# darrenjw/logreg

Hardware: AMD Instinct MI355X
Metric: MCMC iterations/sec x chains for HMC (L=50) on n=200,p=8 (higher is better)
Workload: dtype f32

## Files before the change

logreg_amd/csrc/lr_engine.h:

```cpp
#pragma once

namespace {

template <typename T, int P> lr::ModelArgs<T, P> model_args(const lr_model* m) {
    lr::ModelArgs<T, P> a{};
    a.rows = static_cast<const T*>(m->d_rows);
    a.rows_tw = static_cast<const float*>(m->d_rows_tw);
    a.rows_mf = static_cast<const float*>(m->d_xmf);
    a.ops_mf = static_cast<const unsigned char*>(m->d_xms);
    a.n = m->n;
    for (int j = 0; j < P; ++j) a.prior.inv_var[j] = (T)m->inv_var[j];
    a.prior.lprior_const = m->lprior_const;
    return a;
}

int64_t plan_count(const lr_run_opts* o) { return o->plan_chains > 0 ? (int64_t)o->plan_chains : o->n_chains; }

struct RunSpec {
    int kind;
    double step;
    int l;
    double a[kMaxP], b[kMaxP], c[kMaxP];
};

// ... 48 lines not shown
    const int64_t head = pl.split > 0 ? (pl.split - pos0 < 0 ? 0 : (pl.split - pos0 > C ? C : pl.split - pos0)) : C;
    const bool two = head > 0 && head < C;
    const int64_t head_rounds = pl.mode == lr::MODE_MFMA ? head / ((pl.G == 1 ? 64 : 16) * (int64_t)m->cus) : head * pl.G / 64 / (4LL * m->cus);
    const bool both = two && pl.corun && (rs.kind != lr::KIND_HMC || head_rounds <= 2);
    lr_model::Side* side_slot = nullptr;
    if (both) {
        for (auto& e : m->sides)
            if (e.caller == st) side_slot = &e;
        if (!side_slot) {
            lr_model::Side e{st, nullptr, nullptr, nullptr};
            const bool ok = hipStreamCreateWithFlags(&e.stream, hipStreamNonBlocking) == hipSuccess &&
                            hipEventCreateWithFlags(&e.ev_fork, hipEventDisableTiming) == hipSuccess &&
                            hipEventCreateWithFlags(&e.ev_join, hipEventDisableTiming) == hipSuccess;
            if (!ok) {
                const hipError_t err = hipGetLastError();
                if (e.ev_join) (void)hipEventDestroy(e.ev_join);
                if (e.ev_fork) (void)hipEventDestroy(e.ev_fork);
                if (e.stream) (void)hipStreamDestroy(e.stream);
                return fail(LR_ERR_HIP, "creating the side stream of a two-part launch failed: %s", hipGetErrorString(err));
            }
            m->sides.push_back(e);
            side_slot = &m->sides.back();
        }
        if (hipEventRecord(side_slot->ev_fork, st) != hipSuccess || hipStreamWaitEvent(side_slot->stream, side_slot->ev_fork, 0) != hipSuccess)
            return fail(LR_ERR_HIP, "forking the two-part launch failed: %s", hipGetErrorString(hipGetLastError()));
    }
    for (int part = 0; part < 2; ++part) {
        ca.first = part == 0 ? 0 : head;
        ca.count = part == 0 ? head : C - head;
        if (ca.count <= 0) continue;
        const bool side = both && part == 1;
        lr::LaunchCfg cfg{part == 0 ? pl.mode : pl.mode2, part == 0 ? pl.G : pl.G2, part == 0 ? pl.R : pl.R2, rs.kind, side ? side_slot->stream : st,
                          part == 0 || pl.mode2 == lr::MODE_MIXED ? pl.lds_bytes : 0, m->dbg.residency_cap && !side ? m->cus : 0};
        const int rc = m->table->launch_chain(&cfg, ca.count, &ma, &ca);
        if (rc != 0) return fail(rc == -3 ? LR_ERR_UNSUPPORTED : LR_ERR_HIP, "chain launch failed (%d): %s", rc,
                                 hipGetErrorString(hipGetLastError()));
    }
    if (both) {
        if (hipEventRecord(side_slot->ev_join, side_slot->stream) != hipSuccess || hipStreamWaitEvent(st, side_slot->ev_join, 0) != hipSuccess)
            return fail(LR_ERR_HIP, "joining the two-part launch failed: %s", hipGetErrorString(hipGetLastError()));
    }
    return LR_OK;
}

template <typename T, int P>
int setup_tall(lr_model* m, const Plan& pl, hipStream_t st, int64_t C, int64_t Cp, lr::TallArgs<T, P>* pa) {
    lr::TallArgs<T, P>& a = *pa;
    a = lr::TallArgs<T, P>{};
    const int RS = pl.G;
    auto align = [](size_t b) { return (b + 255) & ~(size_t)255; };
    const size_t vec = align((size_t)C * P * sizeof(T)), dbl = align((size_t)C * sizeof(double));
    const InteriorPlan ip = plan_interior(m, Cp);
    const int RS_i = ip.RS_i, rs_waves = ip.waves;
    const int64_t slice_len_i = ip.slice_len_i;
    const int RSmax = RS_i > RS ? RS_i : RS;
    const size_t pg = align((size_t)RSmax * C * P * sizeof(T)), cv = align((size_t)2 * P * sizeof(T));
    const size_t need = 4 * vec + 2 * dbl + align((size_t)C * 4) + pg + align((size_t)RS * C * sizeof(double)) +
                        (RS_i > 0 && (m->P > 32 || rs_waves == 16) ? 2 * vec + pg : 0) + cv;
    lr_model::Ws* slot = nullptr;
    for (auto& e : m->ws)
        if (e.stream == st) slot = &e;
    if (!slot) {
        if (m->ws.size() >= 16) {
            if (hipDeviceSynchronize() != hipSuccess) return fail(LR_ERR_HIP, "hipDeviceSynchronize failed");
            for (auto& e : m->ws)
                if (e.p) (void)hipFree(e.p);
            m->ws.clear();
// ... 254 lines not shown
```

logreg_amd/csrc/lr_kernels.h:

```cpp
#pragma once
#include <type_traits>

#include "lr_device.h"
#include "lr_stamps.h"

namespace lr {

enum Kind { KIND_RWMH = 0, KIND_MALA = 1, KIND_HMC = 2, KIND_UL = 3 };
enum Mode { MODE_REG = 0, MODE_LDS = 1, MODE_GLOBAL = 2, MODE_MFMA = 3, MODE_STEPWISE = 4, MODE_MIXED = 5 };

template <typename T, int P> struct ModelArgs {
    const T* rows;
    const float* rows_tw;
    const float* rows_mf;
    const unsigned char* ops_mf;
    int64_t n;
    Prior<T, P> prior;
};

template <typename T> struct EvalArgs {
    const T* beta;
    int64_t C;
    int p;
    T* ll;
    T* lprior;
    T* lpost;
    T* grad;
};

template <typename T, int P> struct ChainArgs {
    T* state;
    double* lp_state;
    T* out;
    uint32_t* accepts;
    int64_t C;
    int64_t first, count;
    int64_t chain_offset;
    int64_t iters, thin;
    int64_t iter_offset;
    uint64_t seed;
    int p;
    int l;
    T step;
    T a[P], b[P], c[P];
    T d[P], e[P];
    StatsArgs stats;
    int interior_bf16;
};

template <typename T, int P, int G, int MODE, int R> struct RowsOf {
    using type = StridedRows<T, P, G>;
};
template <typename T, int P, int G, int R> struct RowsOf<T, P, G, MODE_REG, R> {
    using type = RegRows<T, P, R, G>;
};
template <int P, int G, int R> struct RowsOf<float, P, G, MODE_REG, R> {
    using type = RegRowPairs<P, R, G>;
};
template <typename T, int P, int R> struct RowsOf<T, P, 1, MODE_GLOBAL, R> {
    using type = ScalarRows<T, P>;
};
template <int R> struct RowsOf<float, 4, 1, MODE_GLOBAL, R> { using type = ScalarRowPairs<4>; };
template <int R> struct RowsOf<float, 8, 1, MODE_GLOBAL, R> { using type = ScalarRowPairs<8>; };
template <int R> struct RowsOf<float, 16, 1, MODE_GLOBAL, R> { using type = ScalarRowPairs<16>; };

template <typename T, int P, int G, int MODE, int R>
__device__ __forceinline__ typename RowsOf<T, P, G, MODE, R>::type make_rows(const ModelArgs<T, P>& m, int gl,
                                                                             T* smem) {
    typename RowsOf<T, P, G, MODE, R>::type rows;
    if constexpr (MODE == MODE_REG) {
        rows.load(m.rows, m.n, gl);
    } else if constexpr (MODE == MODE_LDS) {
        constexpr int LD = P + kLdsRowPad<T>;
        const int64_t tot = m.n * P;
        for (int64_t i = threadIdx.x; i < tot; i += blockDim.x) smem[(i / P) * LD + (i % P)] = m.rows[i];
        __syncthreads();
        rows.base = smem;
        rows.n = m.n;
        rows.gl = gl;
        rows.ld = LD;
// ... 775 lines not shown
```

logreg_amd/csrc/lr_mfma.h:

```cpp
#pragma once
#include <type_traits>

#include "lr_kernels.h"

namespace lr {

typedef float f32x4 __attribute__((ext_vector_type(4)));

typedef float mf_f32x2 __attribute__((ext_vector_type(2)));
typedef __bf16 mf_bf16x2 __attribute__((ext_vector_type(2)));
typedef __bf16 mf_bf16x8 __attribute__((ext_vector_type(8)));
typedef short mf_s16x4 __attribute__((ext_vector_type(4)));
typedef uint32_t mf_u32x2 __attribute__((ext_vector_type(2)));
typedef uint32_t mf_u32x4 __attribute__((ext_vector_type(4)));
__device__ __forceinline__ uint32_t mf_pack_rne(float a, float b) {
    return __builtin_bit_cast(uint32_t, __builtin_convertvector(mf_f32x2{a, b}, mf_bf16x2));
}
__device__ __forceinline__ float mf_hi_f32(uint32_t packed) { return __builtin_bit_cast(float, packed << 16); }

template <int P, typename Src> __device__ __forceinline__ float mf_row_or_zero(const Src* __restrict__ rows, int64_t n, int64_t row, int coord) {
    const float v = (float)rows[(row < n ? row : n - 1) * P + coord];
    return row < n ? v : 0.0f;
}

template <int P> constexpr int mf_image_floats();
template <int P, int S, bool VALUE>
__device__ __forceinline__ void mf_eval_stream(const float* __restrict__ rows, const float* __restrict__ image, int64_t n, int wave, int lane,
                                               int ntile_live, const float (&q)[P / 4], float (&gl)[P / 4], float& vsum) {
    constexpr int NC = P / 4, NG = (NC + 3) / 4, HG = NC < 4 ? NC : 4;
    const int c = lane & 15, k = lane >> 4;
    const int rp = c & 3, kp = c >> 2;
    float bs[NC];
#pragma unroll
    for (int h = 0; h < NC; ++h) bs[h] = q[h] * ExpScale<float>::k;
    f32x4 ga[NG], gb[NG];
#pragma unroll
    for (int g = 0; g < NG; ++g) ga[g] = gb[g] = f32x4{0, 0, 0, 0};
    float v = 0.0f;
    int pad = 0;
    constexpr int TB = P <= 8 ? 4 : 2;
// ... 49 lines not shown
                    ga[g] = __builtin_amdgcn_mfma_f32_16x16x4f32(cg[i][g][2], w[2], ga[g], 0, 0, 0);
                    gb[g] = __builtin_amdgcn_mfma_f32_16x16x4f32(cg[i][g][3], w[3], gb[g], 0, 0, 0);
                }
            }
        }
#pragma unroll
        for (int i = 0; i < TB; ++i) {
#pragma unroll
            for (int h = 0; h < NC; ++h) ca[i][h] = na[i][h];
#pragma unroll
            for (int g = 0; g < NG; ++g)
#pragma unroll
                for (int s2 = 0; s2 < 4; ++s2) cg[i][g][s2] = ng[i][g][s2];
        }
    }
#pragma unroll
    for (int h = 0; h < NC; ++h) gl[h] = ga[h >> 2][h & 3] + gb[h >> 2][h & 3];
    if constexpr (VALUE) vsum = (v + (float)pad) * ExpScale<float>::inv;
}

template <int P, int NTW, int S, bool END_MEM = false> struct MfmaRows {
    static constexpr int NC = P / 4;
    static constexpr int NU = NC / 2;
    static constexpr int NG = (NC + 3) / 4;
    static constexpr int HG = NC < 4 ? NC : 4;
    float xa[END_MEM ? 1 : NTW][NC];
    float xg[END_MEM ? 1 : NTW][NG][4];
    const float* rows_ = nullptr;
    const float* image = nullptr;
    int64_t n_ = 0;
    int wave_ = 0, lane_ = 0;
    int pad_rows;
    static constexpr int NPAIR = (NTW + 1) / 2;
    mf_u32x4 xe[NTW][NU];
    mf_u32x4 xq[NPAIR][NU];
    int ntile_live;

    template <typename Src> __device__ __forceinline__ void load(const Src* __restrict__ rows, int64_t n, int wave, int lane) {
        const int c = lane & 15, k = lane >> 4;
        const int rp = c & 3, kp = c >> 2;
        pad_rows = 0;
        if constexpr (END_MEM) {
            if constexpr (std::is_same<Src, float>::value) rows_ = rows;
            n_ = n;
            wave_ = wave;
            lane_ = lane;
        } else {
#pragma unroll
            for (int t = 0; t < NTW; ++t) {
                const int64_t base = 16 * ((int64_t)t * S + wave);
                const int64_t ra = base + c;
#pragma unroll
                for (int h = 0; h < NC; ++h) xa[t][h] = mf_row_or_zero<P>(rows, n, ra, k + 4 * h);
#pragma unroll
                for (int s = 0; s < 4; ++s) {
                    const int64_t rg = base + 4 * k + s;
#pragma unroll
                    for (int g = 0; g < NG; ++g) xg[t][g][s] = rp < HG ? mf_row_or_zero<P>(rows, n, rg, kp + 4 * (rp < HG ? rp : 0) + 16 * g) : 0.0f;
                    if (rg >= n) ++pad_rows;
                }
            }
        }
        auto piece = [&](int64_t row, int coord, int lo) {
            const float x = mf_row_or_zero<P>(rows, n, row, coord);
            const uint32_t h = mf_pack_rne(x, x) & 0xFFFFu;
            if (!lo) return h;
            return mf_pack_rne(x - mf_hi_f32(h), 0.0f) & 0xFFFFu;
        };
        ntile_live = 0;
#pragma unroll
        for (int t = 0; t < NTW; ++t) {
            const int64_t base = 16 * ((int64_t)t * S + wave);
            if (base < n) ntile_live = t + 1;
#pragma unroll
            for (int u = 0; u < NU; ++u) {
                uint32_t hl[2];
#pragma unroll
                for (int h = 0; h < 2; ++h) {
                    const float xs = mf_row_or_zero<P>(rows, n, base + c, k + 8 * u + 4 * h) * ExpScale<float>::k;
                    const uint32_t hi = mf_pack_rne(xs, xs) & 0xFFFFu;
                    hl[h] = hi | (mf_pack_rne(0.0f, xs - mf_hi_f32(hi)) & 0xFFFF0000u);
                }
                xe[t][u] = mf_u32x4{hl[0], hl[0], hl[1], hl[1]};
            }
        }
        const int grp = c >> 2, el = c & 3;
        const int gcoord = grp + 4 * (el >> 1), glo = el & 1;
#pragma unroll
        for (int pi = 0; pi < NPAIR; ++pi) {
#pragma unroll
            for (int u = 0; u < NU; ++u) {
                uint32_t v[8];
#pragma unroll
                for (int sl = 0; sl < 8; ++sl) {
                    const int t = 2 * pi + (sl >> 2);
                    const int64_t row = 16 * ((int64_t)t * S + wave) + 4 * k + (sl & 3);
                    v[sl] = t < NTW ? piece(row, gcoord + 8 * u, glo) : 0u;
                }
                xq[pi][u] = mf_u32x4{v[0] | (v[1] << 16), v[2] | (v[3] << 16), v[4] | (v[5] << 16), v[6] | (v[7] << 16)};
            }
        }
    }

    template <int NPL> __device__ __forceinline__ void eval_bf16(const float (&q)[NC], float (&gl)[NC]) const {
        static_assert(NPL >= 1 && NPL <= NPAIR, "pairs");
        mf_u32x4 bb[NU];
#pragma unroll
        for (int u = 0; u < NU; ++u) {
            const uint32_t ha = mf_pack_rne(q[2 * u], q[2 * u]), hb = mf_pack_rne(q[2 * u + 1], q[2 * u + 1]);
            const float la = q[2 * u] - mf_hi_f32(ha), lb = q[2 * u + 1] - mf_hi_f32(hb);
            bb[u] = mf_u32x4{ha, mf_pack_rne(la, la), hb, mf_pack_rne(lb, lb)};
        }
        constexpr int NT = 2 * NPL < NTW ? 2 * NPL : NTW;
        auto eta = [&](int t) {
            f32x4 acc = {0, 0, 0, 0};
#pragma unroll
            for (int u = 0; u < NU; ++u)
                acc = __builtin_amdgcn_mfma_f32_16x16x32_bf16(__builtin_bit_cast(mf_bf16x8, xe[t][u]), __builtin_bit_cast(mf_bf16x8, bb[u]), acc, 0, 0, 0);
            return acc;
        };
        f32x4 e[2 * NPL];
        e[0] = eta(0);
        if constexpr (NT > 1) e[1] = eta(1);
        if constexpr (S == 1) __builtin_amdgcn_sched_barrier(0);
        f32x4 gacc[NU];
#pragma unroll
        for (int u = 0; u < NU; ++u) gacc[u] = f32x4{0, 0, 0, 0};
#pragma unroll
        for (int pi = 0; pi < NPL; ++pi) {
            uint32_t wq[4] = {0u, 0u, 0u, 0u};
            if (2 * pi + 2 < NT) e[2 * pi + 2] = eta(2 * pi + 2);
            if (2 * pi + 3 < NT) e[2 * pi + 3] = eta(2 * pi + 3);
            if constexpr (S == 1) __builtin_amdgcn_sched_barrier(0);
#pragma unroll
            for (int T = 0; T < 2; ++T) {
                const int t = 2 * pi + T;
                if (t < NT) {
                    const mf_f32x2 d0 = mf_f32x2{__builtin_amdgcn_exp2f(e[t][0]), __builtin_amdgcn_exp2f(e[t][1])} + mf_f32x2{1.0f, 1.0f};
                    const mf_f32x2 d1 = mf_f32x2{__builtin_amdgcn_exp2f(e[t][2]), __builtin_amdgcn_exp2f(e[t][3])} + mf_f32x2{1.0f, 1.0f};
                    wq[2 * T] = mf_pack_rne(fast_rcp(d0.x), fast_rcp(d0.y));
                    wq[2 * T + 1] = mf_pack_rne(fast_rcp(d1.x), fast_rcp(d1.y));
                }
            }
            const mf_u32x4 wv = {wq[0], wq[1], wq[2], wq[3]};
#pragma unroll
            for (int u = 0; u < NU; ++u)
                gacc[u] = __builtin_amdgcn_mfma_f32_16x16x32_bf16(__builtin_bit_cast(mf_bf16x8, xq[pi][u]), __builtin_bit_cast(mf_bf16x8, wv), gacc[u], 0, 0, 0);
            if constexpr (S == 1) __builtin_amdgcn_sched_barrier(0);
        }
#pragma unroll
        for (int u = 0; u < NU; ++u) {
            gl[2 * u] = gacc[u][0] + gacc[u][1];
            gl[2 * u + 1] = gacc[u][2] + gacc[u][3];
        }
    }

    template <bool VALUE>
    __device__ __forceinline__ void eval(const float (&q)[NC], float (&gl)[NC], float& vsum) const {
        if constexpr (END_MEM) {
            mf_eval_stream<P, S, VALUE>(rows_, image, n_, wave_, lane_, ntile_live, q, gl, vsum);
            return;
        }
        float bs[NC];
#pragma unroll
        for (int h = 0; h < NC; ++h) bs[h] = q[h] * ExpScale<float>::k;
        f32x4 ga[NG], gb[NG];
#pragma unroll
        for (int g = 0; g < NG; ++g) ga[g] = gb[g] = f32x4{0, 0, 0, 0};
        float v = 0.0f;
#pragma unroll
        for (int t = 0; t < NTW; ++t) {
            f32x4 e = {0, 0, 0, 0};
#pragma unroll
            for (int h = 0; h < NC; ++h) e = __builtin_amdgcn_mfma_f32_16x16x4f32(xa[t][h], bs[h], e, 0, 0, 0);
            float w[4];
#pragma unroll
            for (int r = 0; r < 4; ++r) {
                const float tr = VALUE ? min_keep_nan(e[r], 100.0f) : e[r];
                const float d = 1.0f + __builtin_amdgcn_exp2f(tr);
                w[r] = fast_rcp(d);
                if constexpr (VALUE) v += tr - __builtin_amdgcn_logf(d);
            }
#pragma unroll
            for (int g = 0; g < NG; ++g) {
                ga[g] = __builtin_amdgcn_mfma_f32_16x16x4f32(xg[t][g][0], w[0], ga[g], 0, 0, 0);
                gb[g] = __builtin_amdgcn_mfma_f32_16x16x4f32(xg[t][g][1], w[1], gb[g], 0, 0, 0);
                ga[g] = __builtin_amdgcn_mfma_f32_16x16x4f32(xg[t][g][2], w[2], ga[g], 0, 0, 0);
                gb[g] = __builtin_amdgcn_mfma_f32_16x16x4f32(xg[t][g][3], w[3], gb[g], 0, 0, 0);
            }
        }
#pragma unroll
        for (int h = 0; h < NC; ++h) gl[h] = ga[h >> 2][h & 3] + gb[h >> 2][h & 3];
        if constexpr (VALUE) vsum = (v + (float)pad_rows) * ExpScale<float>::inv;
    }
};

template <int P> constexpr int mf_image_floats() { return P / 4 + 4 * ((P / 4 + 3) / 4); }
template <int P> inline void mf_image_prepare(const float* rows, int64_t n, float* out) {
    constexpr int NC = P / 4, NG = (NC + 3) / 4, HG = NC < 4 ? NC : 4, F = mf_image_floats<P>();
    const int64_t tiles = (n + 15) / 16;
    for (int64_t T = 0; T < tiles; ++T)
        for (int lane = 0; lane < 64; ++lane) {
            const int c = lane & 15, k = lane >> 4, rp = c & 3, kp = c >> 2;
            float* o = out + ((size_t)T * 64 + lane) * F;
            const int64_t ra = 16 * T + c;
            for (int h = 0; h < NC; ++h) o[h] = ra < n ? rows[ra * P + k + 4 * h] : 0.0f;
            for (int g = 0; g < NG; ++g)
                for (int s = 0; s < 4; ++s) {
                    const int64_t rg = 16 * T + 4 * k + s;
                    o[NC + 4 * g + s] = (rg < n && rp < HG) ? rows[rg * P + kp + 4 * rp + 16 * g] : 0.0f;
                }
        }
}

extern __shared__ __attribute__((aligned(16))) unsigned char lr_mfma_dyn_smem[];
template <int P, int S, bool GLOBAL = false> struct MfmaRowsLds {
    static constexpr int NC = P / 4, NU = NC / 2, NG = (NC + 3) / 4, HG = NC < 4 ? NC : 4;
    static constexpr int NPAIR = 1;
    static constexpr int PADP = GLOBAL ? 4 : 0;
    static __host__ __device__ constexpr size_t bytes_per_wave(int64_t ntw) {
        return (size_t)((ntw + 1) / 2 + PADP) * 2 * NU * 64 * 8 + (size_t)((ntw + 1) / 2 + PADP) * NU * 64 * 16;
    }
    const float* rows;
    const float* image;
    int64_t n;
    int wave, lane, ntw, ntile_live;
    mf_u32x2* xe;
    mf_u32x4* xq;

    __device__ __forceinline__ void attach(const float* __restrict__ rows_, int64_t n_, int wave_, int lane_, unsigned char* store) {
        rows = rows_;
        n = n_;
        wave = wave_;
        lane = lane_;
        const int64_t tiles = (n + 15) / 16;
        ntw = (int)((tiles + S - 1) / S);
        const int npair = (ntw + 1) / 2 + PADP;
        unsigned char* base = store + (size_t)wave * bytes_per_wave(ntw);
        xq = reinterpret_cast<mf_u32x4*>(base);
        xe = reinterpret_cast<mf_u32x2*>(base + (size_t)npair * NU * 64 * 16);
        const int64_t live = (tiles - wave + S - 1) / S;
        ntile_live = (int)(live < 0 ? 0 : live);
    }
    __device__ __forceinline__ void load(const float* __restrict__ rows_, int64_t n_, int wave_, int lane_) {
        attach(rows_, n_, wave_, lane_, lr_mfma_dyn_smem);
        build();
    }
    __device__ __forceinline__ void build() {
        const int c = lane & 15, k = lane >> 4;
        const int npair = (ntw + 1) / 2 + PADP;
        auto piece = [&](int64_t row, int coord, int lo) {
// ... 3 lines not shown
            return mf_pack_rne(x - mf_hi_f32(h), 0.0f) & 0xFFFFu;
        };
        for (int t = 0; t < 2 * npair; ++t) {
            const int64_t row0 = t < ntw ? 16 * ((int64_t)t * S + wave) : n;
#pragma unroll
            for (int u = 0; u < NU; ++u) {
                uint32_t hl[2];
#pragma unroll
                for (int h = 0; h < 2; ++h) {
                    const float xs = mf_row_or_zero<P>(rows, n, row0 + c, k + 8 * u + 4 * h) * ExpScale<float>::k;
                    const uint32_t hi = mf_pack_rne(xs, xs) & 0xFFFFu;
                    hl[h] = hi | (mf_pack_rne(0.0f, xs - mf_hi_f32(hi)) & 0xFFFF0000u);
                }
                xe[(t * NU + u) * 64 + lane] = mf_u32x2{hl[0], hl[1]};
            }
        }
        const int grp = c >> 2, el = c & 3;
        const int gcoord = grp + 4 * (el >> 1), glo = el & 1;
        for (int pi = 0; pi < npair; ++pi) {
#pragma unroll
            for (int u = 0; u < NU; ++u) {
                uint32_t v[8];
#pragma unroll
                for (int sl = 0; sl < 8; ++sl) {
                    const int t = 2 * pi + (sl >> 2);
                    const int64_t row = 16 * ((int64_t)t * S + wave) + 4 * k + (sl & 3);
                    v[sl] = t < ntw ? piece(row, gcoord + 8 * u, glo) : 0u;
                }
                xq[(pi * NU + u) * 64 + lane] = mf_u32x4{v[0] | (v[1] << 16), v[2] | (v[3] << 16), v[4] | (v[5] << 16), v[6] | (v[7] << 16)};
            }
        }
    }

    template <int NPL> __device__ __forceinline__ void eval_bf16(const float (&q)[NC], float (&gl)[NC]) const {
        mf_u32x4 bb[NU];
#pragma unroll
        for (int u = 0; u < NU; ++u) {
            const uint32_t ha = mf_pack_rne(q[2 * u], q[2 * u]), hb = mf_pack_rne(q[2 * u + 1], q[2 * u + 1]);
            const float la = q[2 * u] - mf_hi_f32(ha), lb = q[2 * u + 1] - mf_hi_f32(hb);
            bb[u] = mf_u32x4{ha, mf_pack_rne(la, la), hb, mf_pack_rne(lb, lb)};
        }
        f32x4 gacc[NU];
#pragma unroll
        for (int u = 0; u < NU; ++u) gacc[u] = f32x4{0, 0, 0, 0};
        const int npl = (ntile_live + 1) >> 1;
        auto pair_work = [&](int pi) {
            mf_u32x2 he[2][NU];
            mf_u32x4 hq[NU];
#pragma unroll
            for (int T = 0; T < 2; ++T)
#pragma unroll
                for (int u = 0; u < NU; ++u) he[T][u] = xe[((2 * pi + T) * NU + u) * 64 + lane];
#pragma unroll
            for (int u = 0; u < NU; ++u) hq[u] = xq[(pi * NU + u) * 64 + lane];
            uint32_t wq[4];
#pragma unroll
            for (int T = 0; T < 2; ++T) {
                f32x4 e = {0, 0, 0, 0};
#pragma unroll
                for (int u = 0; u < NU; ++u) {
                    const mf_u32x4 av = {he[T][u][0], he[T][u][0], he[T][u][1], he[T][u][1]};
                    e = __builtin_amdgcn_mfma_f32_16x16x32_bf16(__builtin_bit_cast(mf_bf16x8, av), __builtin_bit_cast(mf_bf16x8, bb[u]), e, 0, 0, 0);
                }
                const mf_f32x2 d0 = mf_f32x2{__builtin_amdgcn_exp2f(e[0]), __builtin_amdgcn_exp2f(e[1])} + mf_f32x2{1.0f, 1.0f};
                const mf_f32x2 d1 = mf_f32x2{__builtin_amdgcn_exp2f(e[2]), __builtin_amdgcn_exp2f(e[3])} + mf_f32x2{1.0f, 1.0f};
                wq[2 * T] = mf_pack_rne(fast_rcp(d0.x), fast_rcp(d0.y));
                wq[2 * T + 1] = mf_pack_rne(fast_rcp(d1.x), fast_rcp(d1.y));
// ... 48 lines not shown
                fetch(p0 + 2, tb);
                work(p0, ta);
                fetch(p0 + 4, ta);
                work(p0 + 2, tb);
            }
        } else {
            int pi = 0;
            for (; pi + 1 < npl; pi += 2) {
                pair_work(pi);
                pair_work(pi + 1);
            }
            if (pi < npl) pair_work(pi);
        }
#pragma unroll
        for (int u = 0; u < NU; ++u) {
            gl[2 * u] = gacc[u][0] + gacc[u][1];
            gl[2 * u + 1] = gacc[u][2] + gacc[u][3];
        }
    }

    template <bool VALUE>
    __device__ __forceinline__ void eval(const float (&q)[NC], float (&gl)[NC], float& vsum) const {
        mf_eval_stream<P, S, VALUE>(rows, image, n, wave, lane, ntile_live, q, gl, vsum);
    }
};

template <int N, typename F> __device__ __forceinline__ void for_pair_count(int n, F&& f) {
    if constexpr (N <= 1) {
        f(std::integral_constant<int, 1>{});
    } else {
        if (n >= N) f(std::integral_constant<int, N>{});
        else for_pair_count<N - 1>(n, f);
    }
}

template <typename T> __device__ __forceinline__ T ksum(T v) { return swap32_sum(swap16_sum(v)); }

template <int P, int S>
__global__ void __launch_bounds__(64 * S) k_mfma_image_build(const float* rows, int64_t n, unsigned char* store) {
    MfmaRowsLds<P, S, true> r;
    r.attach(rows, n, threadIdx.x >> 6, threadIdx.x & 63, store);
    r.build();
}

template <int P, int NTW, int S, int KIND>
__global__ void __launch_bounds__((S == 1 ? 256 : 64 * S)) k_chain_mfma(ModelArgs<float, P> m, ChainArgs<float, P> a) {
    constexpr int NC = P / 4;
    constexpr int SW = S == 1 ? 4 : S;
    __shared__ float red[2][SW][64][NC];
    __shared__ double redv[SW][64];
    const int lane = threadIdx.x & 63, wave = __builtin_amdgcn_readfirstlane(threadIdx.x >> 6);
    const int c = lane & 15, k = lane >> 4;
    const int64_t tile0 = S == 1 ? ((int64_t)blockIdx.x * 4 + wave) * 16 : (int64_t)blockIdx.x * 16;
    int64_t chain = a.first + tile0 + c;
    const bool live = chain < a.first + a.count;
    if (!live) chain = a.first + a.count - 1;
    const bool writer = live && (S == 1 || wave == 0);
    const uint64_t gchain = (uint64_t)(a.chain_offset + chain);

    constexpr bool kEndMem = KIND == KIND_HMC && NTW > 0 && NTW * P >= 256;
    using Rows = std::conditional_t<NTW == 0, MfmaRowsLds<P, S, false>,
                                    std::conditional_t<NTW < 0, MfmaRowsLds<P, S, true>, MfmaRows<P, (NTW <= 0 ? 1 : NTW), S, kEndMem>>>;
    Rows rows;
    if constexpr (NTW < 0) {
        const size_t skip = S == 8 ? 4 * MfmaRowsLds<P, 4, true>::bytes_per_wave((int64_t)(((m.n + 15) / 16 + 3) / 4)) : 0;
        rows.attach(m.rows, m.n, wave, lane, const_cast<unsigned char*>(m.ops_mf) + skip);
    }
    else rows.load(m.rows, m.n, S == 1 ? 0 : wave, lane);
    if constexpr (NTW <= 0 || kEndMem) rows.image = m.rows_mf;

    auto pick = [&](const float (&v)[P], int h) {
        const float lo = k == 0 ? v[4 * h] : v[4 * h + 1], hi = k == 2 ? v[4 * h + 2] : v[4 * h + 3];
        return k < 2 ? lo : hi;
    };
    float inv_var[NC], ka[NC], kb[NC], kc[NC], x[NC], g[NC];
#pragma unroll
    for (int h = 0; h < NC; ++h) {
        inv_var[h] = pick(m.prior.inv_var, h);
        ka[h] = pick(a.a, h);
        kb[h] = pick(a.b, h);
        kc[h] = pick(a.c, h);
        const int j = k + 4 * h;
        x[h] = j < a.p ? a.state[chain * a.p + j] : 0.0f;
    }

    int step_parity = 0;
    auto combine = [&](float (&gl)[NC]) {
#pragma unroll
        for (int h = 0; h < NC; ++h) red[step_parity][wave][lane][h] = gl[h];
        __syncthreads();
#pragma unroll
        for (int h = 0; h < NC; ++h) {
            float q4[SW / 4];
#pragma unroll
            for (int w = 0; w < SW; w += 4)
                q4[w / 4] = (red[step_parity][w][lane][h] + red[step_parity][w + 1][lane][h]) +
                            (red[step_parity][w + 2][lane][h] + red[step_parity][w + 3][lane][h]);
            float tot = q4[0];
#pragma unroll
            for (int w = 1; w < SW / 4; ++w) tot += q4[w];
            gl[h] = tot;
        }
    };
    auto evaluate = [&](auto want_value, const float (&q)[NC], float (&grad)[NC], double& ll) {
        constexpr bool VALUE = decltype(want_value)::value;
        float gl[NC], vs = 0.0f;
        rows.template eval<VALUE>(q, gl, vs);
        if constexpr (S > 1) {
            if constexpr (VALUE) redv[wave][lane] = (double)vs;
            combine(gl);
            double dv = 0;
            if constexpr (VALUE) {
#pragma unroll
                for (int w = 0; w < SW; w += 4) dv += (redv[w][lane] + redv[w + 1][lane]) + (redv[w + 2][lane] + redv[w + 3][lane]);
                __syncthreads();
            }
            step_parity ^= 1;
            if constexpr (VALUE) ll = ksum(dv);
        } else {
            if constexpr (VALUE) ll = ksum((double)vs);
        }
#pragma unroll
        for (int h = 0; h < NC; ++h) grad[h] = gl[h] - q[h] * inv_var[h];
    };
    auto evaluate_interior = [&](auto npl, const float (&q)[NC], float (&grad)[NC]) {
        float gl[NC];
        rows.template eval_bf16<decltype(npl)::value>(q, gl);
        if constexpr (S > 1) {
            combine(gl);
            step_parity ^= 1;
        }
#pragma unroll
        for (int h = 0; h < NC; ++h) grad[h] = gl[h] - q[h] * inv_var[h];
    };
    using True = std::integral_constant<bool, true>;
    using False = std::integral_constant<bool, false>;
    auto lprior_of = [&](const float (&q)[NC]) {
        float acc = q[NC - 1] * q[NC - 1] * inv_var[NC - 1];
#pragma unroll
        for (int h = NC - 2; h >= 0; --h) acc = fma_t(q[h] * q[h], inv_var[h], acc);
        return m.prior.lprior_const - 0.5 * (double)ksum(acc);
    };

    double lp;
    uint32_t nacc = 0;
    {
        double ll0 = 0;
        if constexpr (KIND == KIND_HMC) {
            evaluate(True{}, x, g, ll0);
            lp = ll0 + lprior_of(x);
        } else if constexpr (KIND == KIND_MALA) {
            evaluate(False{}, x, g, ll0);
            lp = a.lp_state[chain];
        } else if constexpr (KIND == KIND_UL) {
            evaluate(False{}, x, g, ll0);
            lp = 0;
        } else {
            lp = a.lp_state[chain];
        }
    }

    for (int64_t it = 0; it < a.iters; ++it) {
        for (int64_t jt = 0; jt < a.thin; ++jt) {
            const uint64_t iter = (uint64_t)(a.iter_offset + it * a.thin + jt);
// ... 44 lines not shown
                    lprp = lprior_of(xp);
                    logr = (llp + lprp) - lp;
                } else if constexpr (KIND == KIND_MALA) {
                    float advx[NC];
#pragma unroll
                    for (int h = 0; h < NC; ++h) {
                        advx[h] = fma_t(ka[h], g[h], x[h]);
                        xp[h] = fma_t(kb[h], z[h], advx[h]);
                    }
                    evaluate(True{}, xp, gp, llp);
                    lprp = lprior_of(xp);
                    float dq = 0.0f;
#pragma unroll
                    for (int h = 0; h < NC; ++h) {
                        const float advp = fma_t(ka[h], gp[h], xp[h]);
                        const float d1 = x[h] - advp, d2 = xp[h] - advx[h];
                        dq = fma_t(kc[h], d1 * d1 - d2 * d2, dq);
                    }
                    logr = (llp + lprp) - lp - 0.5 * (double)ksum(dq);
                } else {
                    float pm[NC];
                    float k0 = 0.0f;
#pragma unroll
                    for (int h = 0; h < NC; ++h) {
                        pm[h] = z[h] * ka[h];
                        k0 = fma_t(pm[h] * pm[h], kc[h], k0);
                        xp[h] = x[h];
                        gp[h] = g[h];
                    }
                    const float heps = 0.5f * a.step;
#pragma unroll
                    for (int h = 0; h < NC; ++h) pm[h] = fma_t(heps, gp[h], pm[h]);
                    if (a.interior_bf16) {
                        for_pair_count<Rows::NPAIR>((rows.ntile_live + 1) >> 1, [&](auto npl) {
                            for (int i = 0; i < a.l - 1; ++i) {
#pragma unroll
                                for (int h = 0; h < NC; ++h) xp[h] = fma_t(kb[h], pm[h], xp[h]);
                                evaluate_interior(npl, xp, gp);
#pragma unroll
                                for (int h = 0; h < NC; ++h) pm[h] = fma_t(a.step, gp[h], pm[h]);
                            }
                        });
                    } else {
                        for (int i = 0; i < a.l - 1; ++i) {
#pragma unroll
                            for (int h = 0; h < NC; ++h) xp[h] = fma_t(kb[h], pm[h], xp[h]);
                            double d0;
                            evaluate(False{}, xp, gp, d0);
#pragma unroll
                            for (int h = 0; h < NC; ++h) pm[h] = fma_t(a.step, gp[h], pm[h]);
                        }
                    }
#pragma unroll
                    for (int h = 0; h < NC; ++h) xp[h] = fma_t(kb[h], pm[h], xp[h]);
                    evaluate(True{}, xp, gp, llp);
                    lprp = lprior_of(xp);
                    float k1 = 0.0f;
#pragma unroll
                    for (int h = 0; h < NC; ++h) {
                        pm[h] = fma_t(heps, gp[h], pm[h]);
                        k1 = fma_t(pm[h] * pm[h], kc[h], k1);
                    }
                    logr = ((llp + lprp) - lp) - 0.5 * (double)ksum(k1 - k0);
                }
                const bool acc = logu < logr;
                if (acc) {
                    ++nacc;
                    lp = llp + lprp;
                }
#pragma unroll
                for (int h = 0; h < NC; ++h) {
                    x[h] = acc ? xp[h] : x[h];
                    if constexpr (KIND != KIND_RWMH) g[h] = acc ? gp[h] : g[h];
                }
            }
        }
        if (a.out && writer) {
            float* o = a.out + (it * a.C + chain) * a.p;
#pragma unroll
            for (int h = 0; h < NC; ++h)
                if (k + 4 * h < a.p) o[k + 4 * h] = x[h];
        }
        if (a.stats.buf && writer) {
            const int64_t idx = a.stats.first + it, sb = idx / a.stats.batch, sk = idx - sb * a.stats.batch;
            const double inv = 1.0 / (double)(sk + 1);
            double* s = a.stats.buf + ((sb * a.C + chain) * 2) * a.p;
#pragma unroll
            for (int h = 0; h < NC; ++h)
                if (k + 4 * h < a.p) stats_fold(s + k + 4 * h, s + a.p + k + 4 * h, sk, inv, (double)x[h]);
        }
    }
    if (writer) {
#pragma unroll
        for (int h = 0; h < NC; ++h)
            if (k + 4 * h < a.p) a.state[chain * a.p + k + 4 * h] = x[h];
        if (k == 0) {
            if (a.accepts) a.accepts[chain] += nacc;
            if constexpr (KIND == KIND_RWMH || KIND == KIND_MALA) a.lp_state[chain] = lp;
        }
    }
}

}
```

logreg_amd/csrc/lr_mfma_f64.h:

```cpp
#pragma once
#include "lr_kernels.h"
#include "lr_mfma.h"

namespace lr {

template <int NTW>
__global__ void __launch_bounds__(256) k_chain_mfma_f64(ModelArgs<double, 8> m, ChainArgs<double, 8> a) {
    constexpr int P = 8, NC = 2;
    extern __shared__ __attribute__((aligned(16))) unsigned char smem_raw[];
    double* const srows = reinterpret_cast<double*>(smem_raw);
    const int lane = threadIdx.x & 63, wave = __builtin_amdgcn_readfirstlane(threadIdx.x >> 6);
    const int c = lane & 15, k = lane >> 4;
    const int64_t tile0 = ((int64_t)blockIdx.x * 4 + wave) * 16;
    int64_t chain = a.first + tile0 + c;
    const bool live = chain < a.first + a.count;
    if (!live) chain = a.first + a.count - 1;
    const uint64_t gchain = (uint64_t)(a.chain_offset + chain);
    {
        const int64_t tot = m.n * P;
        for (int64_t i = threadIdx.x; i < tot; i += blockDim.x) srows[i] = m.rows[i];
        __syncthreads();
    }
    MfmaRows<P, NTW, 1> rows;
    rows.load(m.rows, m.n, 0, lane);
// ... 45 lines not shown
    {
        double ll0 = 0;
        evaluate(True{}, x, g, ll0);
        lp = ll0 + lprior_of(x);
    }
    const double heps = 0.5 * a.step;
    for (int64_t it = 0; it < a.iters; ++it) {
        for (int64_t jt = 0; jt < a.thin; ++jt) {
            const uint64_t iter = (uint64_t)(a.iter_offset + it * a.thin + jt);
            double z[NC], logu;
            {
                const U4 w4 = philox4x32_10((uint32_t)gchain, (uint32_t)iter, (uint32_t)(iter >> 32), k < 2 ? (uint32_t)k : TAG_UNIFORM,
                                            (uint32_t)a.seed, (uint32_t)(a.seed >> 32));
                double nrm[4];
                box_muller(w4.x, w4.y, nrm[0], nrm[1]);
                box_muller(w4.z, w4.w, nrm[2], nrm[3]);
                logu = from(c + 32, log(u01<double>(w4.x)));
#pragma unroll
                for (int h = 0; h < NC; ++h) {
                    const double e0 = from(c + 16 * h, nrm[0]), e1 = from(c + 16 * h, nrm[1]);
                    const double e2 = from(c + 16 * h, nrm[2]), e3 = from(c + 16 * h, nrm[3]);
                    z[h] = k < 2 ? (k == 0 ? e0 : e1) : (k == 2 ? e2 : e3);
                }
            }
            double pm[NC], xp[NC], gp[NC], k0 = 0.0;
#pragma unroll
            for (int h = 0; h < NC; ++h) {
                pm[h] = z[h] * ka[h];
                k0 = __builtin_fma(pm[h] * pm[h], kc[h], k0);
                xp[h] = x[h];
                pm[h] = __builtin_fma(heps, g[h], pm[h]);
            }
            if (a.interior_bf16) {
                for_pair_count<MfmaRows<P, NTW, 1>::NPAIR>((rows.ntile_live + 1) >> 1, [&](auto npl) {
                    for (int i = 0; i < a.l - 1; ++i) {
                        float qf[NC], gl[NC];
#pragma unroll
                        for (int h = 0; h < NC; ++h) {
                            xp[h] = __builtin_fma(kb[h], pm[h], xp[h]);
                            qf[h] = (float)xp[h];
                        }
                        rows.template eval_bf16<decltype(npl)::value>(qf, gl);
#pragma unroll
                        for (int h = 0; h < NC; ++h) pm[h] = __builtin_fma(a.step, __builtin_fma(-xp[h], inv_var[h], (double)gl[h]), pm[h]);
                    }
                });
            } else {
                for (int i = 0; i < a.l - 1; ++i) {
#pragma unroll
                    for (int h = 0; h < NC; ++h) xp[h] = __builtin_fma(kb[h], pm[h], xp[h]);
                    double d0;
                    evaluate(False{}, xp, gp, d0);
#pragma unroll
                    for (int h = 0; h < NC; ++h) pm[h] = __builtin_fma(a.step, gp[h], pm[h]);
                }
            }
#pragma unroll
            for (int h = 0; h < NC; ++h) xp[h] = __builtin_fma(kb[h], pm[h], xp[h]);
            double llp = 0;
            evaluate(True{}, xp, gp, llp);
            const double lprp = lprior_of(xp);
            double k1 = 0.0;
#pragma unroll
            for (int h = 0; h < NC; ++h) {
                pm[h] = __builtin_fma(heps, gp[h], pm[h]);
                k1 = __builtin_fma(pm[h] * pm[h], kc[h], k1);
            }
            const double logr = ((llp + lprp) - lp) - 0.5 * ksum(k1 - k0);
            const bool acc = logu < logr;
            if (acc) {
                ++nacc;
                lp = llp + lprp;
            }
#pragma unroll
            for (int h = 0; h < NC; ++h) {
// ... 29 lines not shown
```

logreg_amd/csrc/lr_stamps.h:

```cpp
#pragma once

#ifdef LR_STAMPS
#define LR_STAMP_FIELDS                                                                                     \
    unsigned long long* stamps;                                 \
    int stamp_slot;                                                                                         \
    int dbg;
#define LR_STAMP_AT(a, k)                                                                                                    \
    (a).stamps[((((size_t)(a).stamp_slot * (gridDim.x * gridDim.y) + blockIdx.y * gridDim.x + blockIdx.x) * 16) + (threadIdx.x >> 6)) * 16 + (k)]
#define LR_STAMP(a, k) do { if ((a).stamps && (threadIdx.x & 63) == 0) LR_STAMP_AT(a, k) = __builtin_amdgcn_s_memrealtime(); } while (0)
#define LR_STAMP_CLK(a, k) do { if ((a).stamps && (threadIdx.x & 63) == 0) LR_STAMP_AT(a, k) = __builtin_amdgcn_s_memtime(); } while (0)
#define LR_DBG(a, bit) (((a).dbg >> (bit)) & 1)
#define LR_RS16_PHASES_BEGIN unsigned long long ph[4] = {0, 0, 0, 0}, tp = __builtin_amdgcn_s_memtime();
#define LR_RS16_PHASE(k) do { const unsigned long long tn_ = __builtin_amdgcn_s_memtime(); ph[k] += tn_ - tp; tp = tn_; } while (0)
#define LR_RS16_PHASES_REPORT(kind, its)                                                                                                       \
    if (blockIdx.x == 0 && threadIdx.x == 0 && (its) >= 100)                                                                                   \
        printf("k_chain_rs16 kind %d, %lld iterations, shader cycles per iteration: draws %.1f, proposal + evaluation %.1f, accept %.1f, loop %.1f\n", \
               (kind), (long long)(its), (double)ph[0] / (its), (double)ph[1] / (its), (double)ph[2] / (its), (double)ph[3] / (its));
#define LR_TRAJ_PHASES_BEGIN unsigned long long tph[5] = {0, 0, 0, 0, 0}, ttp = __builtin_amdgcn_s_memtime(); const unsigned long long tt0 = ttp;
#define LR_TRAJ_PHASE(k) do { const unsigned long long tn_ = __builtin_amdgcn_s_memtime(); tph[k] += tn_ - ttp; ttp = tn_; } while (0)
#define LR_TRAJ_PHASES_REPORT(a)                                                                         \
    if ((a).stamps && (threadIdx.x & 63) == 0) {                                                         \
        for (int k_ = 0; k_ < 5; ++k_) LR_STAMP_AT(a, 8 + k_) = tph[k_];                                 \
        LR_STAMP_AT(a, 7) = __builtin_amdgcn_s_memtime() - tt0;                                         \
    }
#ifdef LR_TRAJ2_EXP
#define LR_TRAJ_EXP(bit) (((LR_TRAJ2_EXP) >> (bit)) & 1)
#else
#define LR_TRAJ_EXP(bit) 0
#endif
#else
#define LR_STAMP_FIELDS
#define LR_TRAJ_EXP(bit) 0
#define LR_TRAJ_PHASES_BEGIN
#define LR_TRAJ_PHASE(k) do { } while (0)
#define LR_TRAJ_PHASES_REPORT(a)
#define LR_STAMP(a, k) do { } while (0)
#define LR_STAMP_CLK(a, k) do { } while (0)
#define LR_DBG(a, bit) 0
#define LR_RS16_PHASES_BEGIN
#define LR_RS16_PHASE(k) do { } while (0)
#define LR_RS16_PHASES_REPORT(kind, its)
#endif

#if defined(LR_STAMPS_HOST)
#ifdef LR_STAMPS
namespace {
constexpr int kStampSlots = 64, kStampWgs = 512;
int g_stamp_slot = 0;
unsigned long long* g_stamp_buf = nullptr;
constexpr size_t kStampBytes = (size_t)kStampSlots * kStampWgs * 16 * 16 * sizeof(unsigned long long);
unsigned long long* stamp_buffer() {
    if (!g_stamp_buf && (hipMalloc(&g_stamp_buf, kStampBytes) != hipSuccess || hipMemset(g_stamp_buf, 0, kStampBytes) != hipSuccess))
        g_stamp_buf = nullptr;
    return g_stamp_buf;
}
}
#define LR_STAMPS_ARM(a)                                                             \
    do {                                                                             \
        (a).stamps = g_stamp_slot < kStampSlots ? stamp_buffer() : nullptr;          \
        (a).stamp_slot = g_stamp_slot++;                                             \
        const char* e_ = getenv("LOGREG_DEBUG_EXP");                                 \
        (a).dbg = e_ ? atoi(e_) : 0;                                                 \
    } while (0)
#define LR_STAMPS_DISARM(a) do { (a).stamps = nullptr; } while (0)
extern "C" __attribute__((visibility("default"))) int lr_debug_read_stamps(unsigned long long* out, int* slots, int* wgs) {
    if (slots) *slots = kStampSlots;
    if (wgs) *wgs = kStampWgs;
    if (!g_stamp_buf || !out) return 0;
// ... 12 lines not shown
```

Before: 224.6 million.

## Deal rows contiguously across waves and skip dead lanes in final MFMA tile

Replaces the strided tile-to-wave row assignment with a contiguous block deal (MfmaDeal), so each wave holds a balanced run of rows. The interior HMC evaluation is specialised on the exact tile count and the number of live registers in the last partial tile, skipping exp/rcp work for padded rows. It also adds optional timing-stamp instrumentation, which compiles away in normal builds. The cost is more template instantiations and a permuted row order in the partial tile.

```diff
diff --git a/logreg_amd/csrc/lr_engine.h b/logreg_amd/csrc/lr_engine.h
--- a/logreg_amd/csrc/lr_engine.h
+++ b/logreg_amd/csrc/lr_engine.h
@@ -104,7 +104,9 @@
         const bool side = both && part == 1;
         lr::LaunchCfg cfg{part == 0 ? pl.mode : pl.mode2, part == 0 ? pl.G : pl.G2, part == 0 ? pl.R : pl.R2, rs.kind, side ? side_slot->stream : st,
                           part == 0 || pl.mode2 == lr::MODE_MIXED ? pl.lds_bytes : 0, m->dbg.residency_cap && !side ? m->cus : 0};
+        LR_STAMPS_ARM(ca);
         const int rc = m->table->launch_chain(&cfg, ca.count, &ma, &ca);
+        LR_STAMPS_DISARM(ca);
         if (rc != 0) return fail(rc == -3 ? LR_ERR_UNSUPPORTED : LR_ERR_HIP, "chain launch failed (%d): %s", rc,
                                  hipGetErrorString(hipGetLastError()));
     }
diff --git a/logreg_amd/csrc/lr_kernels.h b/logreg_amd/csrc/lr_kernels.h
--- a/logreg_amd/csrc/lr_kernels.h
+++ b/logreg_amd/csrc/lr_kernels.h
@@ -46,6 +46,7 @@
     T d[P], e[P];
     StatsArgs stats;
     int interior_bf16;
+    LR_STAMP_FIELDS
 };
 
 template <typename T, int P, int G, int MODE, int R> struct RowsOf {
diff --git a/logreg_amd/csrc/lr_mfma.h b/logreg_amd/csrc/lr_mfma.h
--- a/logreg_amd/csrc/lr_mfma.h
+++ b/logreg_amd/csrc/lr_mfma.h
@@ -2,10 +2,14 @@
 #include <type_traits>
 
 #include "lr_kernels.h"
+#include "lr_mfma_deal.h"
 
 namespace lr {
 
 typedef float f32x4 __attribute__((ext_vector_type(4)));
+struct MfNoPhase {
+    __device__ __forceinline__ void operator()(int) const {}
+};
 
 typedef float mf_f32x2 __attribute__((ext_vector_type(2)));
 typedef __bf16 mf_bf16x2 __attribute__((ext_vector_type(2)));
@@ -121,9 +125,13 @@
     int wave_ = 0, lane_ = 0;
     int pad_rows;
     static constexpr int NPAIR = (NTW + 1) / 2;
+    static constexpr int NTD = NTW, NLR = 4;
     mf_u32x4 xe[NTW][NU];
     mf_u32x4 xq[NPAIR][NU];
     int ntile_live;
+    int nt_bf, live_bf;
+    __device__ __forceinline__ int interior_tiles() const { return nt_bf; }
+    __device__ __forceinline__ int interior_live() const { return live_bf; }
 
     template <typename Src> __device__ __forceinline__ void load(const Src* __restrict__ rows, int64_t n, int wave, int lane) {
         const int c = lane & 15, k = lane >> 4;
@@ -158,15 +166,20 @@
         };
         ntile_live = 0;
 #pragma unroll
+        for (int t = 0; t < NTW; ++t)
+            if (16 * ((int64_t)t * S + wave) < n) ntile_live = t + 1;
+        const MfmaDeal deal(n, S);
+        nt_bf = deal.tiles(wave);
+        live_bf = deal.live_regs(wave);
+#pragma unroll
         for (int t = 0; t < NTW; ++t) {
-            const int64_t base = 16 * ((int64_t)t * S + wave);
-            if (base < n) ntile_live = t + 1;
+            const int64_t ra = deal.row_at(wave, t, c);
 #pragma unroll
             for (int u = 0; u < NU; ++u) {
                 uint32_t hl[2];
 #pragma unroll
                 for (int h = 0; h < 2; ++h) {
-                    const float xs = mf_row_or_zero<P>(rows, n, base + c, k + 8 * u + 4 * h) * ExpScale<float>::k;
+                    const float xs = mf_row_or_zero<P>(rows, n, ra, k + 8 * u + 4 * h) * ExpScale<float>::k;
                     const uint32_t hi = mf_pack_rne(xs, xs) & 0xFFFFu;
                     hl[h] = hi | (mf_pack_rne(0.0f, xs - mf_hi_f32(hi)) & 0xFFFF0000u);
                 }
@@ -183,16 +196,17 @@
 #pragma unroll
                 for (int sl = 0; sl < 8; ++sl) {
                     const int t = 2 * pi + (sl >> 2);
-                    const int64_t row = 16 * ((int64_t)t * S + wave) + 4 * k + (sl & 3);
-                    v[sl] = t < NTW ? piece(row, gcoord + 8 * u, glo) : 0u;
+                    v[sl] = t < NTW ? piece(deal.row_at(wave, t, 4 * k + (sl & 3)), gcoord + 8 * u, glo) : 0u;
                 }
                 xq[pi][u] = mf_u32x4{v[0] | (v[1] << 16), v[2] | (v[3] << 16), v[4] | (v[5] << 16), v[6] | (v[7] << 16)};
             }
         }
     }
 
-    template <int NPL> __device__ __forceinline__ void eval_bf16(const float (&q)[NC], float (&gl)[NC]) const {
-        static_assert(NPL >= 1 && NPL <= NPAIR, "pairs");
+    template <int NT, int LR, typename PH = MfNoPhase>
+    __device__ __forceinline__ void eval_bf16(const float (&q)[NC], float (&gl)[NC], PH phase = PH{}) const {
+        static_assert(NT >= 1 && NT <= NTW && LR >= 1 && LR <= 4, "tiles, live registers");
+        constexpr int NPL = (NT + 1) / 2;
         mf_u32x4 bb[NU];
 #pragma unroll
         for (int u = 0; u < NU; ++u) {
@@ -200,7 +214,6 @@
             const float la = q[2 * u] - mf_hi_f32(ha), lb = q[2 * u + 1] - mf_hi_f32(hb);
             bb[u] = mf_u32x4{ha, mf_pack_rne(la, la), hb, mf_pack_rne(lb, lb)};
         }
-        constexpr int NT = 2 * NPL < NTW ? 2 * NPL : NTW;
         auto eta = [&](int t) {
             f32x4 acc = {0, 0, 0, 0};
 #pragma unroll
@@ -211,6 +224,7 @@
         f32x4 e[2 * NPL];
         e[0] = eta(0);
         if constexpr (NT > 1) e[1] = eta(1);
+        phase(0);
         if constexpr (S == 1) __builtin_amdgcn_sched_barrier(0);
         f32x4 gacc[NU];
 #pragma unroll
@@ -220,21 +234,30 @@
             uint32_t wq[4] = {0u, 0u, 0u, 0u};
             if (2 * pi + 2 < NT) e[2 * pi + 2] = eta(2 * pi + 2);
             if (2 * pi + 3 < NT) e[2 * pi + 3] = eta(2 * pi + 3);
+            phase(0);
             if constexpr (S == 1) __builtin_amdgcn_sched_barrier(0);
 #pragma unroll
             for (int T = 0; T < 2; ++T) {
                 const int t = 2 * pi + T;
                 if (t < NT) {
-                    const mf_f32x2 d0 = mf_f32x2{__builtin_amdgcn_exp2f(e[t][0]), __builtin_amdgcn_exp2f(e[t][1])} + mf_f32x2{1.0f, 1.0f};
-                    const mf_f32x2 d1 = mf_f32x2{__builtin_amdgcn_exp2f(e[t][2]), __builtin_amdgcn_exp2f(e[t][3])} + mf_f32x2{1.0f, 1.0f};
-                    wq[2 * T] = mf_pack_rne(fast_rcp(d0.x), fast_rcp(d0.y));
-                    wq[2 * T + 1] = mf_pack_rne(fast_rcp(d1.x), fast_rcp(d1.y));
-                }
-            }
+                    const int live = t == NT - 1 ? LR : 4;
+#pragma unroll
+                    for (int j = 0; j < 2; ++j) {
+                        if (live >= 2 * j + 2) {
+                            const mf_f32x2 d = mf_f32x2{__builtin_amdgcn_exp2f(e[t][2 * j]), __builtin_amdgcn_exp2f(e[t][2 * j + 1])} + mf_f32x2{1.0f, 1.0f};
+                            wq[2 * T + j] = mf_pack_rne(fast_rcp(d.x), fast_rcp(d.y));
+                        } else if (live == 2 * j + 1) {
+                            wq[2 * T + j] = mf_pack_rne(fast_rcp(__builtin_amdgcn_exp2f(e[t][2 * j]) + 1.0f), 0.0f);
+                        }
+                    }
+                }
+            }
+            phase(1);
             const mf_u32x4 wv = {wq[0], wq[1], wq[2], wq[3]};
 #pragma unroll
             for (int u = 0; u < NU; ++u)
                 gacc[u] = __builtin_amdgcn_mfma_f32_16x16x32_bf16(__builtin_bit_cast(mf_bf16x8, xq[pi][u]), __builtin_bit_cast(mf_bf16x8, wv), gacc[u], 0, 0, 0);
+            phase(2);
             if constexpr (S == 1) __builtin_amdgcn_sched_barrier(0);
         }
 #pragma unroll
@@ -242,6 +265,7 @@
             gl[2 * u] = gacc[u][0] + gacc[u][1];
             gl[2 * u + 1] = gacc[u][2] + gacc[u][3];
         }
+        phase(2);
     }
 
     template <bool VALUE>
@@ -305,7 +329,9 @@
 extern __shared__ __attribute__((aligned(16))) unsigned char lr_mfma_dyn_smem[];
 template <int P, int S, bool GLOBAL = false> struct MfmaRowsLds {
     static constexpr int NC = P / 4, NU = NC / 2, NG = (NC + 3) / 4, HG = NC < 4 ? NC : 4;
-    static constexpr int NPAIR = 1;
+    static constexpr int NTD = 1, NLR = 1;
+    __device__ __forceinline__ int interior_tiles() const { return 1; }
+    __device__ __forceinline__ int interior_live() const { return 1; }
     static constexpr int PADP = GLOBAL ? 4 : 0;
     static __host__ __device__ constexpr size_t bytes_per_wave(int64_t ntw) {
         return (size_t)((ntw + 1) / 2 + PADP) * 2 * NU * 64 * 8 + (size_t)((ntw + 1) / 2 + PADP) * NU * 64 * 16;
@@ -375,7 +401,8 @@
         }
     }
 
-    template <int NPL> __device__ __forceinline__ void eval_bf16(const float (&q)[NC], float (&gl)[NC]) const {
+    template <int NT, int LR, typename PH = MfNoPhase>
+    __device__ __forceinline__ void eval_bf16(const float (&q)[NC], float (&gl)[NC], PH = PH{}) const {
         mf_u32x4 bb[NU];
 #pragma unroll
         for (int u = 0; u < NU; ++u) {
@@ -490,6 +517,9 @@
         if (n >= N) f(std::integral_constant<int, N>{});
         else for_pair_count<N - 1>(n, f);
     }
+}
+template <typename Rows, typename F> __device__ __forceinline__ void for_interior_shape(const Rows& rows, F&& f) {
+    for_pair_count<Rows::NTD>(rows.interior_tiles(), [&](auto nt) { for_pair_count<Rows::NLR>(rows.interior_live(), [&](auto lr) { f(nt, lr); }); });
 }
 
 template <typename T> __device__ __forceinline__ T ksum(T v) { return swap32_sum(swap16_sum(v)); }
@@ -542,6 +572,8 @@
         x[h] = j < a.p ? a.state[chain * a.p + j] : 0.0f;
     }
 
+    LR_TRAJ_PHASES_BEGIN
+    auto phase = [&](int ph_) { (void)ph_; LR_TRAJ_PHASE_FENCED(ph_); };
     int step_parity = 0;
     auto combine = [&](float (&gl)[NC]) {
 #pragma unroll
@@ -581,13 +613,14 @@
 #pragma unroll
         for (int h = 0; h < NC; ++h) grad[h] = gl[h] - q[h] * inv_var[h];
     };
-    auto evaluate_interior = [&](auto npl, const float (&q)[NC], float (&grad)[NC]) {
+    auto evaluate_interior = [&](auto nt, auto lr, const float (&q)[NC], float (&grad)[NC]) {
         float gl[NC];
-        rows.template eval_bf16<decltype(npl)::value>(q, gl);
+        rows.template eval_bf16<decltype(nt)::value, decltype(lr)::value>(q, gl, phase);
         if constexpr (S > 1) {
             combine(gl);
             step_parity ^= 1;
         }
+        phase(3);
 #pragma unroll
         for (int h = 0; h < NC; ++h) grad[h] = gl[h] - q[h] * inv_var[h];
     };
@@ -698,13 +731,15 @@
 #pragma unroll
                     for (int h = 0; h < NC; ++h) pm[h] = fma_t(heps, gp[h], pm[h]);
                     if (a.interior_bf16) {
-                        for_pair_count<Rows::NPAIR>((rows.ntile_live + 1) >> 1, [&](auto npl) {
+                        for_interior_shape(rows, [&](auto nt, auto lr) {
+                            LR_TRAJ_PHASE_SKIP;
                             for (int i = 0; i < a.l - 1; ++i) {
 #pragma unroll
                                 for (int h = 0; h < NC; ++h) xp[h] = fma_t(kb[h], pm[h], xp[h]);
-                                evaluate_interior(npl, xp, gp);
+                                evaluate_interior(nt, lr, xp, gp);
 #pragma unroll
                                 for (int h = 0; h < NC; ++h) pm[h] = fma_t(a.step, gp[h], pm[h]);
+                                phase(4);
                             }
                         });
                     } else {
@@ -765,6 +800,7 @@
             if constexpr (KIND == KIND_RWMH || KIND == KIND_MALA) a.lp_state[chain] = lp;
         }
     }
+    LR_TRAJ_PHASES_REPORT(a)
 }
 
 }
diff --git a/logreg_amd/csrc/lr_mfma_deal.h b/logreg_amd/csrc/lr_mfma_deal.h
--- /dev/null
+++ b/logreg_amd/csrc/lr_mfma_deal.h
@@ -0,0 +1,40 @@
+#pragma once
+#include <cstdint>
+
+#if defined(__HIPCC__) || defined(__CUDACC__)
+#define LR_DEAL_HD __host__ __device__
+#else
+#define LR_DEAL_HD
+#endif
+
+namespace lr {
+
+struct MfmaSlot {
+    int wave, tile, trow;
+};
+
+struct MfmaDeal {
+    int64_t n, m;
+    LR_DEAL_HD MfmaDeal(int64_t n_, int S) : n(n_), m((n_ + S - 1) / S) {}
+    LR_DEAL_HD int64_t first(int w) const { return w * m < n ? w * m : n; }
+    LR_DEAL_HD int rows(int w) const { return (int)(n - first(w) < m ? n - first(w) : m); }
+    LR_DEAL_HD int tiles(int w) const { return (rows(w) + 15) / 16; }
+    LR_DEAL_HD int live_regs(int w) const {
+        const int r = rows(w), rem = r % 16;
+        return r == 0 ? 0 : rem ? (rem + 3) / 4 : 4;
+    }
+    LR_DEAL_HD static int kmajor(int i) { return 4 * (i & 3) + (i >> 2); }
+    LR_DEAL_HD MfmaSlot place(int64_t row) const {
+        const int w = (int)(row / m);
+        const int off = (int)(row - w * m), whole = rows(w) / 16;
+        const int t = off / 16, i = off % 16;
+        return MfmaSlot{w, t, t < whole ? i : kmajor(i)};
+    }
+    LR_DEAL_HD int64_t row_at(int w, int tile, int trow) const {
+        const int r = rows(w), whole = r / 16, i = kmajor(trow);
+        const bool full = tile < whole, held = full | ((tile == whole) & (i < r % 16));
+        return held ? first(w) + 16 * tile + (full ? trow : i) : n;
+    }
+};
+
+}
diff --git a/logreg_amd/csrc/lr_mfma_f64.h b/logreg_amd/csrc/lr_mfma_f64.h
--- a/logreg_amd/csrc/lr_mfma_f64.h
+++ b/logreg_amd/csrc/lr_mfma_f64.h
@@ -101,7 +101,7 @@
                 pm[h] = __builtin_fma(heps, g[h], pm[h]);
             }
             if (a.interior_bf16) {
-                for_pair_count<MfmaRows<P, NTW, 1>::NPAIR>((rows.ntile_live + 1) >> 1, [&](auto npl) {
+                for_interior_shape(rows, [&](auto nt, auto lr) {
                     for (int i = 0; i < a.l - 1; ++i) {
                         float qf[NC], gl[NC];
 #pragma unroll
@@ -109,7 +109,7 @@
                             xp[h] = __builtin_fma(kb[h], pm[h], xp[h]);
                             qf[h] = (float)xp[h];
                         }
-                        rows.template eval_bf16<decltype(npl)::value>(qf, gl);
+                        rows.template eval_bf16<decltype(nt)::value, decltype(lr)::value>(qf, gl);
 #pragma unroll
                         for (int h = 0; h < NC; ++h) pm[h] = __builtin_fma(a.step, __builtin_fma(-xp[h], inv_var[h], (double)gl[h]), pm[h]);
                     }
diff --git a/logreg_amd/csrc/lr_stamps.h b/logreg_amd/csrc/lr_stamps.h
--- a/logreg_amd/csrc/lr_stamps.h
+++ b/logreg_amd/csrc/lr_stamps.h
@@ -18,6 +18,8 @@
                (kind), (long long)(its), (double)ph[0] / (its), (double)ph[1] / (its), (double)ph[2] / (its), (double)ph[3] / (its));
 #define LR_TRAJ_PHASES_BEGIN unsigned long long tph[5] = {0, 0, 0, 0, 0}, ttp = __builtin_amdgcn_s_memtime(); const unsigned long long tt0 = ttp;
 #define LR_TRAJ_PHASE(k) do { const unsigned long long tn_ = __builtin_amdgcn_s_memtime(); tph[k] += tn_ - ttp; ttp = tn_; } while (0)
+#define LR_TRAJ_PHASE_FENCED(k) do { __builtin_amdgcn_sched_barrier(0); LR_TRAJ_PHASE(k); __builtin_amdgcn_sched_barrier(0); } while (0)
+#define LR_TRAJ_PHASE_SKIP do { ttp = __builtin_amdgcn_s_memtime(); } while (0)
 #define LR_TRAJ_PHASES_REPORT(a)                                                                         \
     if ((a).stamps && (threadIdx.x & 63) == 0) {                                                         \
         for (int k_ = 0; k_ < 5; ++k_) LR_STAMP_AT(a, 8 + k_) = tph[k_];                                 \
@@ -34,6 +36,8 @@
 #define LR_TRAJ_PHASES_BEGIN
 #define LR_TRAJ_PHASE(k) do { } while (0)
 #define LR_TRAJ_PHASES_REPORT(a)
+#define LR_TRAJ_PHASE_FENCED(k) do { } while (0)
+#define LR_TRAJ_PHASE_SKIP do { } while (0)
 #define LR_STAMP(a, k) do { } while (0)
 #define LR_STAMP_CLK(a, k) do { } while (0)
 #define LR_DBG(a, bit) 0
```

Result: no change. 224.3 million (-0.1%).
